# ctpeterson/qex

Hardware: AMD Instinct MI355X
Metric: staggered Dslash GFLOP/s + CG iters/s, 32^4 SU(3) fp64, 1/2/4/8 MI355X (higher is better)
Workload: dtype f64

## Files before the change

include/qexhip.h:

```cpp
#ifndef QEXHIP_H
#define QEXHIP_H

#include <stddef.h>

#ifdef __cplusplus
extern "C" {
#endif

typedef struct qexhip_ctx *qexhip_handle;

#define QEXHIP_OK 0
#define QEXHIP_ERR_ARG (-1)
#define QEXHIP_ERR_HIP (-2)
#define QEXHIP_ERR_STATE (-3)
#define QEXHIP_ERR_COMM (-4)
#define QEXHIP_ERR_IO (-5)

#define QEXHIP_EVEN 0
#define QEXHIP_ODD 1
#define QEXHIP_ALL 2

int qexhip_init(qexhip_handle *h, int device, const int latLocal[4],
                const int rankGeom[4], const int rankCoord[4]);
int qexhip_finalize(qexhip_handle h);
// ... 120 lines not shown
int qexhip_fat7_deriv(qexhip_handle h, const double *g, const double *dfl, const double coef[5], const double *dll, double naik, double *d);
int qexhip_hisq_force(qexhip_handle h, const double *g, const double *dsdsu, const double *dsdsul, double *f);
int qexhip_hisq_prepare(qexhip_handle h, const double *g, double *fl, double *ll);
int qexhip_hisq_closure_force(qexhip_handle h, const double *dsdsu, const double *dsdsul, double *f);
int qexhip_hisq_release(qexhip_handle h);
int qexhip_hisq_fermion_force(qexhip_handle h, double *f, const double *const *psi, const double *scale, int n);

int qexhip_stag_solve_xx_batch(qexhip_handle h, int n, double *const *x, const double *const *b, const double *mass,
                               const double *r2req, int maxits, int par_even, int *iters, double *r2_over_b2);
int qexhip_stag_solve_batch(qexhip_handle h, int n, double *const *x, const double *const *b, const double *mass,
                            const double *r2req, int maxits, int *iters, double *r2_over_b2);

int qexhip_stag_links_info(qexhip_handle h, int *nlinks, int *compressed, double *max_dev);
int qexhip_stag_links_storage(qexhip_handle h, int *bytes_per_link, long long *escaped);
int qexhip_link_residual_host(const double *links, int n, unsigned char *escaped, double *row2);
int qexhip_set_option(qexhip_handle h, const char *name, int value);

int qexhip_stag_set_links_hisq(qexhip_handle h, const double *g);
int qexhip_stag_set_links_nhyp(qexhip_handle h, const double *g, double alpha1, double alpha2, double alpha3,
                               const int antiperiodic[4], const int phases[4]);

int qexhip_nhyp_prepare(qexhip_handle h, const double *g, double alpha1, double alpha2, double alpha3, double *fl);
int qexhip_nhyp_force(qexhip_handle h, double *f, const double *chain);
int qexhip_nhyp_release(qexhip_handle h);
int qexhip_nhyp_gauge_force(qexhip_handle h, double *f, double cplaq, double crect, double cadjplaq);
int qexhip_nhyp_fforce(qexhip_handle h, double *f, int n, const double *const *phi, const double *mass, const double *scale,
                       const double *r2req, int maxits, const int antiperiodic[4], const int phases[4], int *iters);
int qexhip_nhyp_fermion_force(qexhip_handle h, double *f, const double *const *psi, const double *scale, int n,
                              const int antiperiodic[4], const int phases[4]);
int qexhip_nhyp_fforce_dev(qexhip_handle h, double *f, int n, const int *phi_ids, const double *mass, const double *scale,
// ... 55 lines not shown
```

qex_amd/__init__.py:

```python
from ._lib import QexHipError, LIB_PATH, lib
from .layout import Layout
from .gauge import setBC, stagPhase, rephase, unit, synthetic_random_su3, synthetic_gaussian_vector
from .staggered import (
    Context, device_count, Staggered, SolverParams, newStag, newStag3, link_residual_host, plaq, gaugeForce, gaugeFlow, gaugeSet, gaugeFlowResident, flowEQ, flowMeasure, gaugeAction, gaugeUpdate, reunit, wline, ploops, s4_gauge, ResidentMD, HisqCoefs, HypCoefs, makeImpLinks, fat7lDeriv, EVEN, ODD, ALL,
    SloppyNone, SloppySingle, SloppyHalf,
)
from .io import loadGauge, loadGaugeSlab, saveGauge, getFileLattice, gaugeFileInfo, writeField, readField, fileMetadata
from .rng import RngField, RngMilc6, MRG32k3a
from .mesons import stagLocalMesons, stagMesons, norm2slice, sft, printLocalMesons, pointSource, wallSource, localMesonTables
```

qex_amd/_lib.py:

```python
import ctypes as C
import os

_HERE = os.path.dirname(os.path.abspath(__file__))
LIB_PATH = os.environ.get("QEXHIP_LIB", os.path.join(_HERE, "libqexhip.so"))
_lib = None

_vp, _ci, _cd = C.c_void_p, C.c_int, C.c_double
_pi, _pd = C.POINTER(C.c_int), C.POINTER(C.c_double)
SYMBOLS = [
    ("qexhip_init", _ci, [C.POINTER(_vp), _ci, _pi, _pi, _pi]),
    ("qexhip_finalize", _ci, [_vp]),
    ("qexhip_device_count", _ci, [_pi]),
    ("qexhip_last_error", C.c_char_p, []),
    ("qexhip_sync", _ci, [_vp]),
    ("qexhip_device_info", _ci, [_vp, C.c_char_p, _ci]),
    ("qexhip_layout_default_inner", _ci, [_pi, _ci, _pi]),
    ("qexhip_layout_simd_map", _ci, [_pi, _pi, _pi]),
    ("qexhip_layout_vec_simd_to_v1", _ci, [_pi, _pi, _vp, _vp]),
    ("qexhip_layout_vec_v1_to_simd", _ci, [_pi, _pi, _vp, _vp]),
    ("qexhip_layout_gauge_simd_to_v1", _ci, [_pi, _pi, C.POINTER(C.c_void_p), _vp]),
    ("qexhip_layout_gauge_v1_to_simd", _ci, [_pi, _pi, _vp, C.POINTER(C.c_void_p)]),
    ("qexhip_comm_unique_id", _ci, [C.c_char_p]),
    ("qexhip_comm_init", _ci, [_vp, C.c_char_p, _ci, _ci]),
    ("qexhip_comm_force_halo", _ci, [_vp, _ci]),
# ... 46 lines not shown
    ("qexhip_plaq", _ci, [_vp, _vp]),
    ("qexhip_gauge_force", _ci, [_vp, _vp, _cd]),
    ("qexhip_wflow", _ci, [_vp, _ci, _cd]),
    ("qexhip_flow_EQ", _ci, [_vp, _ci, _vp]),
    ("qexhip_flow_measure", _ci, [_vp, _vp, _vp]),
    ("qexhip_gauge_force_general", _ci, [_vp, _vp, _cd, _cd, _ci]),
    ("qexhip_wflow_general", _ci, [_vp, _ci, _cd, _cd, _cd, _ci]),
    ("qexhip_fat7", _ci, [_vp, _vp, _pd, _vp, _vp, _cd]),
    ("qexhip_hisq_smear", _ci, [_vp, _vp, _vp, _vp]),
    ("qexhip_nhyp_smear", _ci, [_vp, _vp, _vp, _cd, _cd, _cd]),
    ("qexhip_stag_solve_xx_batch", _ci, [_vp, _ci, _vp, _vp, _vp, _vp, _ci, _ci, _pi, _vp]),
    ("qexhip_stag_solve_batch", _ci, [_vp, _ci, _vp, _vp, _vp, _vp, _ci, _pi, _vp]),
    ("qexhip_stag_links_info", _ci, [_vp, _pi, _pi, _vp]),
    ("qexhip_stag_links_storage", _ci, [_vp, _pi, C.POINTER(C.c_longlong)]),
    ("qexhip_link_residual_host", _ci, [_vp, _ci, _vp, _vp]),
    ("qexhip_set_option", _ci, [_vp, C.c_char_p, _ci]),
    ("qexhip_fat7_deriv", _ci, [_vp, _vp, _vp, _vp, _vp, _cd, _vp]),
    ("qexhip_hisq_force", _ci, [_vp, _vp, _vp, _vp, _vp]),
    ("qexhip_hisq_prepare", _ci, [_vp, _vp, _vp, _vp]),
    ("qexhip_hisq_closure_force", _ci, [_vp, _vp, _vp, _vp]),
    ("qexhip_hisq_release", _ci, [_vp]),
    ("qexhip_hisq_fermion_force", _ci, [_vp, _vp, _vp, _vp, _ci]),
    ("qexhip_stag_set_links_hisq", _ci, [_vp, _vp]),
    ("qexhip_stag_set_links_nhyp", _ci, [_vp, _vp, _cd, _cd, _cd, _pi, _pi]),
    ("qexhip_nhyp_prepare", _ci, [_vp, _vp, _cd, _cd, _cd, _vp]),
    ("qexhip_nhyp_force", _ci, [_vp, _vp, _vp]),
    ("qexhip_nhyp_release", _ci, [_vp]),
    ("qexhip_nhyp_fforce", _ci, [_vp, _vp, _ci, _vp, _vp, _vp, _vp, _ci, _pi, _pi, _pi]),
    ("qexhip_nhyp_gauge_force", _ci, [_vp, _vp, _cd, _cd, _cd]),
    ("qexhip_nhyp_fermion_force", _ci, [_vp, _vp, _vp, _vp, _ci, _pi, _pi]),
# ... 101 lines not shown
```

qex_amd/csrc/api.cpp:

```cpp
#include "qexhip_internal.h"
#include <string>
#include "../../include/qexhip.h"
#include <algorithm>
#include <cstdarg>
#include <cstdlib>
#include <cstring>
#include <vector>

static thread_local char g_err[1024] = "";

void qexhip_set_error(const char *fmt, ...) {
  va_list ap;
  va_start(ap, fmt);
  vsnprintf(g_err, sizeof(g_err), fmt, ap);
  va_end(ap);
}
extern "C" const char *qexhip_last_error(void) { return g_err; }

static bool timer_class_on(const qexhip_ctx *c, const char *name) {
  if (!c->timers_on) return false;
  if (c->timers_on == 2) return strncmp(name, "dslash", 6) == 0;
  if (c->timers_on == 3) return strncmp(name, "dslash", 6) == 0 || strcmp(name, "exchange") == 0 || strcmp(name, "allreduce") == 0;
  return true;
}
// ... 770 lines not shown
extern "C" int qexhip_stag_solve_batch(qexhip_handle c, int n, double *const *x, const double *const *b, const double *mass,
                                       const double *r2req, int maxits, int *iters, double *r2_over_b2) {
  if (!c || !x || !b || !mass || !r2req) return QEXHIP_ERR_ARG;
  HIPCHK(hipSetDevice(c->device));
  return solve_batch_host(c, n, x, b, mass, r2req, maxits, -1, iters, r2_over_b2);
}
extern "C" int qexhip_stag_links_info(qexhip_handle c, int *nlinks, int *compressed, double *max_dev) {
  if (!c) return QEXHIP_ERR_ARG;
  if (nlinks) *nlinks = c->W ? c->ndir : 0;
  if (compressed) *compressed = c->recon;
  if (max_dev) *max_dev = c->recon_dev;
  return 0;
}
extern "C" int qexhip_stag_links_storage(qexhip_handle c, int *bytes_per_link, long long *escaped) {
  if (!c) return QEXHIP_ERR_ARG;
  if (bytes_per_link) *bytes_per_link = !c->W ? 0 : (c->lres ? 108 : (c->recon == 1 ? 96 : (c->recon == 2 ? 112 : 144)));
  if (escaped) *escaped = c->lres_esc;
  return 0;
}
extern "C" int qexhip_link_residual_host(const double *links, int n, unsigned char *escaped, double *row2) {
  if (!links || n < 0) return QEXHIP_ERR_ARG;
  return link_residual_host((const double2 *)links, n, escaped, (double2 *)row2);
}
extern "C" int qexhip_hisq_prepare(qexhip_handle c, const double *g, double *fl, double *ll) {
  if (!c || !g) return QEXHIP_ERR_ARG;
  HIPCHK(hipSetDevice(c->device));
  return hisq_prepare(c, g, fl, ll);
}
extern "C" int qexhip_hisq_closure_force(qexhip_handle c, const double *dsdsu, const double *dsdsul, double *f) {
  if (!c || !dsdsu || !dsdsul || !f) return QEXHIP_ERR_ARG;
  HIPCHK(hipSetDevice(c->device));
  return hisq_closure_force(c, dsdsu, dsdsul, f);
}
extern "C" int qexhip_hisq_fermion_force(qexhip_handle c, double *f, const double *const *psi, const double *scale, int n) {
  if (!c || !f || !psi || !scale) return QEXHIP_ERR_ARG;
  HIPCHK(hipSetDevice(c->device));
  return hisq_fermion_force(c, f, psi, scale, n);
// ... 209 lines not shown
```

qex_amd/csrc/dslash.hip:

```cpp
#include "qexhip_internal.h"
#include "site_index.h"
#include "reduce.h"
#include "fused_sweep.h"
#include <hip/hip_ext.h>
#include <cstring>
#include <algorithm>
#include <chrono>

static double now_us() { return std::chrono::duration<double, std::micro>(std::chrono::steady_clock::now().time_since_epoch()).count(); }

struct DslashArgs {
  Geom g;
  const double2 *W;
  const unsigned long long *S;
  const double2 *in;
  double2 *out;
  const double2 *rin;
  const double2 *xs;
  double ca, cb;
  double sgn;
  double post;
  int parity, c0, c1;
  int d0, d1, nb1;
  const double2 *gh_hi, *gh_lo;
// ... 22 lines not shown
    if (A.swz && !bnd) {
      int per = A.swz >> 3;
      lb = (lb & 7) * per + (lb >> 3);
    }
    int c = A.c0 + lb * 256 + threadIdx.x;
    int clim = A.c1;
    if (FUSED) c = fused_site(A.fs, R, lb, A.c0, A.c1, A.d0, A.d1, clim);
    else if (lb >= A.nb1) { c = A.d0 + (lb - A.nb1) * 256 + threadIdx.x; clim = A.d1; }
    double dotv = 0;
    const bool active = c < clim && !skip;
    const Geom &g = A.g;
    const SiteXYZT s = site_coord(g, c, A.parity);
    const int tu = FUSED ? __builtin_amdgcn_readfirstlane(s.t) : 0;
    double2 acc[3];
    double2 xsv[3];
    constexpr int NLOAD = (RECON == 1 || RECON == 3) ? 6 : (RECON == 2 ? 7 : 9);
    constexpr int LROW = RECON == 3 ? LR_ROW : NLOAD * 64;
    const double2 *w = A.W + (size_t)(c >> 6) * (NDIR * LROW) + (c & 63);
    const unsigned long long *sm = RECON == 1 ? A.S + (size_t)(c >> 6) * NDIR : (RECON == 3 ? A.S + (size_t)(c >> 6) * NDIR * 2 : nullptr);
    const double2 *in_f1 = A.in, *in_b1 = A.in, *in_f3 = A.in, *in_b3 = A.in;
    if (FUSED) {
      in_f1 = tu + 1 >= g.X[3] ? A.gh_hi : A.in;
      in_b1 = tu - 1 < 0 ? A.gh_lo : A.in;
      in_f3 = tu + 3 >= g.X[3] ? A.gh_hi : A.in;
      in_b3 = tu - 3 < 0 ? A.gh_lo : A.in;
    }
    auto pair = [&](const int pr, const bool do_f, const bool do_b) __attribute__((always_inline)) {
      const int mu = pr & 3;
      const int hop = pr >= 4 ? 3 : 1;
      const int pf = nbr_pos<HALO>(g, c, s, mu, hop);
      const int pb = nbr_pos<HALO>(g, c, s, mu, -hop);
      const double2 *wp = w + (size_t)pr * (2 * LROW);
      double2 U[9], W[9], vf[3], vb[3];
      if (do_f) {
// ... 7 lines not shown
#pragma unroll
        for (int k = 0; k < NLOAD; k++) {
          d2v t = __builtin_nontemporal_load((const d2v *)&wp[LROW + k * 64]);
          W[k] = make_double2(t.x, t.y);
        }
      }
      if (RECON == 1) {
        const int lane = c & 63;
        if (do_f) recon_row2<1>(U, (sm[2 * pr] >> lane) & 1ull);
        if (do_b) recon_row2<1>(W, (sm[2 * pr + 1] >> lane) & 1ull);
      } else if (RECON == 3) {
        const int lane = c & 63;
        const size_t fr = ((size_t)(c >> 6) * NDIR + 2 * pr) * 576 + lane;
        if (do_f) recon_row2_res(U, wp - lane, sm + 4 * pr, A.S - 2, fr, lane);
        if (do_b) recon_row2_res(W, wp - lane + LROW, sm + 4 * pr + 2, A.S - 2, fr + 576, lane);
      } else if (RECON == 2) {
        if (do_f) recon_row2<2>(U, false);
        if (do_b) recon_row2<2>(W, false);
      }
      const double2 *srcf = (FUSED && mu == 3) ? (hop == 3 ? in_f3 : in_f1) : A.in;
      const double2 *srcb = (FUSED && mu == 3) ? (hop == 3 ? in_b3 : in_b1) : A.in;
      if (do_f) {
#pragma unroll
        for (int k = 0; k < 3; k++) vf[k] = srcf[vec_off(pf, k)];
      }
      if (do_b) {
#pragma unroll
        for (int k = 0; k < 3; k++) vb[k] = srcb[vec_off(pb, k)];
      }
      if (do_f) mv3<false>(acc, U, vf);
// ... 63 lines not shown
          acc[k].x *= (A.sgn * A.post); acc[k].y *= (A.sgn * A.post);
          if (A.ntstore) {
            d2v t; t.x = acc[k].x; t.y = acc[k].y;
            __builtin_nontemporal_store(t, (d2v *)&A.out[vec_off(c, k)]);
          } else {
            A.out[vec_off(c, k)] = acc[k];
          }
        }
        if (DOT) {
#pragma unroll
          for (int k = 0; k < 3; k++) dotv = fma(xsv[k].x, acc[k].x, fma(xsv[k].y, acc[k].y, dotv));
        }
      }
    }
    if (DOT && !skip && !parked) {
      const int pidx = !FUSED ? (RECON == 3 ? lb : (int)blockIdx.x) : fused_partial_slot(A.fs, R, lb);
      double r = block_sum_256(dotv);
      if (threadIdx.x == 0) A.partials[pidx] = r;
    }
    if (!cleanup) break;
  }
  if (FUSED) fused_finish(A.fs, R);
}

template <int NDIR, bool HALO, bool INIT, bool DOT, int RECON>
__global__ void __launch_bounds__(256) k_dslash(DslashArgs A) { dslash_body<NDIR, HALO, INIT, DOT, RECON, false>(A); }
template <int NDIR, bool INIT, bool DOT, int RECON>
__global__ void __launch_bounds__(256) k_dslash_fused(DslashArgs A) { dslash_body<NDIR, true, INIT, DOT, RECON, true>(A); }

template <class K>
static void launch_timed(qexhip_ctx *c, const char *tname, K kernel, dim3 grid, dim3 block, DslashArgs &A, hipStream_t st) {
// ... 21 lines not shown
#define QX_LAUNCH(R) \
  do { \
    if (HALO && fused) { \
      if (init && dot) launch_timed(c, tname, k_dslash_fused<NDIR, true, true, R>, grid, block, A, st); \
      else if (init) launch_timed(c, tname, k_dslash_fused<NDIR, true, false, R>, grid, block, A, st); \
      else if (dot) launch_timed(c, tname, k_dslash_fused<NDIR, false, true, R>, grid, block, A, st); \
      else launch_timed(c, tname, k_dslash_fused<NDIR, false, false, R>, grid, block, A, st); \
    } else if (init && dot) launch_timed(c, tname, k_dslash<NDIR, HALO, true, true, R>, grid, block, A, st); \
    else if (init) launch_timed(c, tname, k_dslash<NDIR, HALO, true, false, R>, grid, block, A, st); \
    else if (dot) launch_timed(c, tname, k_dslash<NDIR, HALO, false, true, R>, grid, block, A, st); \
    else launch_timed(c, tname, k_dslash<NDIR, HALO, false, false, R>, grid, block, A, st); \
  } while (0)
  if (c->recon == 1) QX_LAUNCH(1);
  else if (c->recon == 2) QX_LAUNCH(2);
  else if constexpr (NDIR == 8) {
    if (c->lres) QX_LAUNCH(3);
    else QX_LAUNCH(0);
  } else QX_LAUNCH(0);
#undef QX_LAUNCH
  A.partials = psave;
  HIPCHK(hipGetLastError());
  return 0;
}

void sweep_plan(const qexhip_ctx *c, int *lo_end_out, int *hi_beg_out, int *overlap_out) {
  const Geom &g = c->g;
  int lo_end = g.depth * g.F; if (lo_end > g.Vh) lo_end = g.Vh;
  int hi_beg = g.Vh - g.depth * g.F; if (hi_beg < lo_end) hi_beg = lo_end;
  const size_t face_bytes = (size_t)g.depth * g.F * 48;
  *lo_end_out = lo_end; *hi_beg_out = hi_beg;
  const int tuned = c->overlap_auto[c->ndir == 16];
// ... 4 lines not shown

int sweep_form(const qexhip_ctx *c, int overlap) {
  if (!overlap || !peer_faces(c)) return 0;
  if (c->opt_hop_split >= 0) return c->opt_hop_split ? 2 : 0;
  const int m = c->form_auto[c->ndir == 16];
  return m >= 0 ? m : 2;
}

static double exchange_estimate_us(const qexhip_ctx *c) {
  const double meas = c->xchg_us[c->ndir == 16];
  if (meas > 0) return meas;
  const double link = (c->emu_link_gbs > 0 ? c->emu_link_gbs : 45.0) * 1e3;
  return 3.0 + (double)c->g.depth * c->g.F * 48.0 / link;
}
double sweep_push_fraction(const qexhip_ctx *c, int interior_sites, int nrhs) {
  const double bsite = c->ndir * (c->recon == 1 ? 96.0 : (c->recon == 2 ? 112.0 : (c->lres ? 108.0 : 144.0))) + 120.0 * nrhs;
  const double t_int = (double)interior_sites * bsite / 5.5e6;
  return t_int > 0 ? std::min(1.0, std::max(0.65, nrhs * exchange_estimate_us(c) / t_int)) : 1.0;
}

static int sweep_fused_ctl(qexhip_ctx *c, int nbnd, FusedCtl *F, int nrhs) {
  if (c->fz_cap < nbnd) {
    HIPCHK(hipStreamSynchronize(c->stream));
    if (c->fz_buf) HIPCHK(hipFree(c->fz_buf));
    c->fz_buf = nullptr; c->fz_cap = 0;
    const int cap = std::max(2 * nbnd, 4096);
    HIPCHK(hipMalloc((void **)&c->fz_buf, (size_t)(256 + cap) * sizeof(unsigned int)));
    HIPCHK(hipMemsetAsync(c->fz_buf, 0, (size_t)(256 + cap) * sizeof(unsigned int), c->stream));
    c->fz_cap = cap;
  }
  F->dec = c->fz_buf; F->ndef = c->fz_buf + 32; F->cl_done = c->fz_buf + 64; F->late = c->fz_buf + 96;
// ... 96 lines not shown
  if (saved < 0) c->overlap_auto[slot] = (best > 0 && v[0] > 0 && best < 0.95 * v[0]) ? 1 : 0;
  for (int k = 0; k < 3; k++) c->overlap_tune_us[slot][k] = v[k] / 10.0;
  return 0;
}

int dslash_sweep(qexhip_ctx *c, DevField &out, DevField &in, int parity, const DslashOpts &o) {
  const Geom &g = c->g;
  if (!c->W) { qexhip_set_error("staggered links not set (qexhip_stag_set_links)"); return -3; }
  DslashArgs A;
  memset(&A, 0, sizeof A);
  A.g = g;
  if (c->recon) {
    A.W = c->Wc + (size_t)parity * g.ntile * c->ndir * (c->recon == 1 ? 384 : 448);
    A.S = c->Ws + (size_t)parity * g.ntile * c->ndir;
  } else if (c->lres) {
    A.W = c->Wc + (size_t)parity * g.ntile * c->ndir * LR_ROW;
    A.S = c->Wm + (size_t)parity * (2 + g.ntile * c->ndir * 2) + 2;
  } else {
    A.W = c->W + (size_t)parity * g.ntile * c->ndir * 576;
    A.S = nullptr;
  }
  A.in = in.par(1 - parity);
  A.out = out.par(parity);
  A.rin = o.rin ? o.rin->par(parity) : nullptr;
  A.xs = o.xs ? o.xs->par(parity) : nullptr;
  A.ca = o.ca; A.cb = o.cb;
  A.sgn = o.neg ? -1.0 : 1.0;
  A.post = o.post;
  A.parity = parity;
  A.partials = c->partials;
  A.done = o.done;
// ... 54 lines not shown
```

qex_amd/csrc/dslash_core.h:

```cpp
#pragma once
#include <hip/hip_runtime.h>
#include "link_residual.h"

typedef double d2v __attribute__((ext_vector_type(2)));

template <bool SUB>
__device__ __forceinline__ void mv3(double2 acc[3], const double2 U[9], const double2 v[3]) {
#pragma unroll
  for (int i = 0; i < 3; i++) {
#pragma unroll
    for (int j = 0; j < 3; j++) {
      if (!SUB) {
        acc[i].x += U[3 * i + j].x * v[j].x;
        acc[i].x -= U[3 * i + j].y * v[j].y;
        acc[i].y += U[3 * i + j].x * v[j].y;
        acc[i].y += U[3 * i + j].y * v[j].x;
      } else {
        acc[i].x -= U[3 * i + j].x * v[j].x;
        acc[i].x += U[3 * i + j].y * v[j].y;
        acc[i].y -= U[3 * i + j].x * v[j].y;
        acc[i].y -= U[3 * i + j].y * v[j].x;
      }
    }
  }
// ... 24 lines not shown
__device__ __forceinline__ void recon_row2_res(double2 U[9], const double2 *row, const unsigned long long *m, const unsigned long long *hdr,
                                               size_t fr, int lane) {
  const uint64_t lo = __builtin_nontemporal_load((const uint64_t *)(row + LR_RES) + lane);
  const uint32_t hi = __builtin_nontemporal_load((const uint32_t *)(row + LR_RES + 32) + lane);
  double2 r2[3];
  lr_decode(U, (m[0] >> lane) & 1ull, lo, hi, r2);
  if ((m[1] >> lane) & 1ull) {
    const double2 *wf = (const double2 *)(uintptr_t)hdr[0] + fr;
#pragma unroll
    for (int k = 0; k < 3; k++) r2[k] = wf[(6 + k) * 64];
  }
#pragma unroll
  for (int k = 0; k < 3; k++) U[6 + k] = r2[k];
}

template <int RECON>
__device__ __forceinline__ void load_link(double2 U[9], const double2 *w, const unsigned long long *sm, int lane) {
  constexpr int NLOAD = RECON == 1 ? 6 : (RECON == 2 ? 7 : 9);
#pragma unroll
  for (int k = 0; k < NLOAD; k++) U[k] = w[k * 64];
  if (RECON == 1) recon_row2<1>(U, (*sm >> lane) & 1ull);
  else if (RECON == 2) recon_row2<2>(U, false);
}
```

qex_amd/csrc/layout.hip:

```cpp
#include <algorithm>
#include <vector>
#include "qexhip_internal.h"
#include "site_index.h"
#include "link_residual.h"
#include <cstring>

int geom_init(Geom &g, const int X[4], int depth, int halo) {
  for (int i = 0; i < 4; i++) {
    if (X[i] < 2 || (X[i] & 1)) { qexhip_set_error("local lattice extents must be even and >= 2 (got %d in dim %d)", X[i], i); return -1; }
    if (X[i] > 1024) { qexhip_set_error("local lattice extents above 1024 are not supported (got %d in dim %d)", X[i], i); return -1; }
    g.X[i] = X[i];
  }
  g.Xh = X[0] / 2;
  g.V = X[0] * X[1] * X[2] * X[3];
  g.Vh = g.V / 2;
  g.F = g.Xh * X[1] * X[2];
  g.ntile = (g.Vh + QEXHIP_TILE - 1) / QEXHIP_TILE;
  g.halo = halo;
  g.depth = halo ? depth : 0;
  if (halo) {
    if (g.F % QEXHIP_TILE) { qexhip_set_error("sharding in t needs X*Y*Z/2 to be a multiple of 64 (got %d)", g.F); return -1; }
    if (X[3] < 3) { qexhip_set_error("sharding in t needs a local t extent >= 3"); return -1; }
    g.gtile = 3 * g.F / QEXHIP_TILE;
  } else {
// ... 196 lines not shown
  bool neg;
  uint64_t lo;
  uint32_t hi;
  const bool ok = lr_encode(u, &neg, &lo, &hi);
  ((uint64_t *)(Wc + row * LR_ROW + LR_RES))[l] = lo;
  ((uint32_t *)(Wc + row * LR_ROW + LR_RES + 32))[l] = hi;
  const unsigned long long sgn = __ballot(neg), esc = __ballot(!ok);
  if (l == 0) {
    unsigned long long *m = Wm + 2 * (row + row / prows + 1);
    m[0] = sgn;
    m[1] = esc;
    if (esc) atomicAdd(nesc, (unsigned int)__popcll(esc));
  }
}

int link_residual_host(const double2 *u, long n, unsigned char *escaped, double2 *row2) {
  for (long i = 0; i < n; i++) {
    bool neg;
    uint64_t lo;
    uint32_t hi;
    const bool ok = lr_encode(u + 9 * i, &neg, &lo, &hi);
    if (escaped) escaped[i] = !ok;
    if (row2) lr_decode(u + 9 * i, neg, lo, hi, row2 + 3 * i);
  }
  return 0;
}

int links_compress(qexhip_ctx *c) {
  const Geom &g = c->g;
  c->links_gen++;
  c->recon = 0;
  c->lres = 0; c->lres_esc = 0;
  if (!c->opt_recon || !c->W) return 0;
  const size_t nrows = (size_t)2 * g.ntile * c->ndir;
  if (c->Wc_rows < nrows) {
    if (c->Wc) HIPCHK(hipFree(c->Wc));
    if (c->Ws) HIPCHK(hipFree(c->Ws));
    HIPCHK(hipMalloc((void **)&c->Wc, nrows * 448 * sizeof(double2)));
// ... 4 lines not shown
  const unsigned nblk = (unsigned)((nrows * 64 + 255) / 256);
  for (int fmt = 1; fmt <= 2; fmt++) {
    if (fmt == 2 && c->opt_recon == 1) break;
    HIPCHK(hipMemsetAsync(flag, 0, sizeof(unsigned int), c->stream));
    if (fmt == 1) k_links_compress<1><<<nblk, 256, 0, c->stream>>>(nrows, c->W, c->Wc, c->Ws, flag);
    else k_links_compress<2><<<nblk, 256, 0, c->stream>>>(nrows, c->W, c->Wc, c->Ws, flag);
    HIPCHK(hipGetLastError());
    unsigned int bits = 0;
    HIPCHK(hipMemcpyAsync(&bits, flag, sizeof(bits), hipMemcpyDeviceToHost, c->stream));
    HIPCHK(hipStreamSynchronize(c->stream));
    float dev;
    memcpy(&dev, &bits, sizeof(dev));
    if (fmt == 1 || dev <= 5e-14f) c->recon_dev = dev;
    if (dev <= 5e-14f) { c->recon = fmt; break; }
  }
  if (!c->recon && c->opt_lossless && c->ndir == 8) {
    if (!c->Wm || c->Wm_rows < nrows) {
      if (c->Wm) HIPCHK(hipFree(c->Wm));
      c->Wm = nullptr; c->Wm_rows = 0;
      HIPCHK(hipMalloc((void **)&c->Wm, (nrows + 2) * 2 * sizeof(unsigned long long)));
      c->Wm_rows = nrows;
    }
    const size_t prows = nrows / 2;
    HIPCHK(hipMemsetAsync(flag, 0, sizeof(unsigned int), c->stream));
    k_links_residual<<<nblk, 256, 0, c->stream>>>(nrows, prows, c->W, c->Wc, c->Wm, flag);
    HIPCHK(hipGetLastError());
    unsigned int nesc = 0;
    HIPCHK(hipMemcpyAsync(&nesc, flag, sizeof(nesc), hipMemcpyDeviceToHost, c->stream));
    const unsigned long long hdr[2][2] = {{(unsigned long long)(uintptr_t)c->W, 0}, {(unsigned long long)(uintptr_t)(c->W + prows * 576), 0}};
    for (int p = 0; p < 2; p++) HIPCHK(hipMemcpyAsync(c->Wm + p * 2 * (prows + 1), hdr[p], sizeof hdr[p], hipMemcpyHostToDevice, c->stream));
    HIPCHK(hipStreamSynchronize(c->stream));
    c->lres_esc = nesc;
    if ((double)nesc <= 0.01 * (double)(nrows * 64)) c->lres = 1;
  }
  return 0;
}

__global__ void __launch_bounds__(256) k_links_from_nat(Geom g, const double2 *__restrict__ N, double2 *W, int ndir, int dbase, int hop) {
  int i = blockIdx.x * 256 + threadIdx.x;
  if (i >= g.V) return;
  int p = i >= g.Vh, c = i - p * g.Vh;
  SiteXYZT s = site_coord(g, c, p);
  double2 *w = W + ((size_t)p * g.ntile + (c >> 6)) * ndir * 576 + (c & 63);
  for (int mu = 0; mu < 4; mu++) {
    const double2 *U = N + (((size_t)p * g.etile + (c >> 6)) * 4 + mu) * 576 + (c & 63);
    double2 *wf = w + (size_t)(dbase + 2 * mu) * 576;
    for (int k = 0; k < 9; k++) wf[k * 64] = U[k * 64];
    int cb;
// ... 167 lines not shown
```

qex_amd/csrc/qexhip_internal.h:

```cpp
#pragma once
#include <hip/hip_runtime.h>
#include <cstdint>
#include <cstdio>
#include <string>
#include <vector>
#include <map>

#define QEXHIP_TILE 64

struct Geom {
  int X[4];
  int Xh;
  int V, Vh;
  int F;
  int ntile;
  int depth;
  int gtile;
  int etile;
  int halo;
};

__host__ __device__ inline size_t vec_off(int pos, int colour) {
  return (size_t)(pos >> 6) * 192 + (size_t)colour * 64 + (size_t)(pos & 63);
}
// ... 68 lines not shown
  int next_field = 1;
  double *stage = nullptr; size_t stage_bytes = 0;
  double *partials = nullptr; int npartials = 0;
  int part2_off = 0;
  double *dscal = nullptr;
  CgScal *cg = nullptr;
  struct { int valid = 0; const double2 *x = nullptr; int par_even = 0; double m2 = 0; int k = 0; } cg_resume;
  int cg_r2parts = 0;
  double *hist = nullptr; int histcap = 0;
  void *pinned = nullptr;
  int wk[WK_SLOTS]{0};
  int timers_on = 0;
  std::map<std::string, TimerSlot> timers;
  double2 *Wc = nullptr; unsigned long long *Ws = nullptr; size_t Wc_rows = 0; int recon = 0; double recon_dev = 0;
  unsigned long long *Wm = nullptr; size_t Wm_rows = 0; int lres = 0; long long lres_esc = 0;
  int opt_lossless = 1;
  int opt_batch_multi = 0;
  int opt_multi_reduce = 0;
  int opt_force_pair = 1;
  int opt_obs_clover = 1;
  int opt_hop_split = -1;
  int opt_fused_spin_us = -1;
  int ranks_share_device = 0;
  int hybrid_sums = 0;
  unsigned int *fz_buf = nullptr; int fz_cap = 0;
  const double2 *bnd_out_on_cstream = nullptr;
  double xchg_us[2]{0, 0};
  int form_auto[2]{-1, -1};
  int opt_chain_overlap = 1;
  int opt_smear_ca = 1;
  int opt_flow_exp = 1;
// ... 38 lines not shown
  ScopedTimer(qexhip_ctx *c_, const char *name, hipStream_t st_);
  ~ScopedTimer();
};
int timers_collect(qexhip_ctx *c);
bool timer_event_pair(qexhip_ctx *c, const char *name, hipEvent_t *e0, hipEvent_t *e1);

int geom_init(Geom &g, const int X[4], int depth, int halo);
int field_alloc(qexhip_ctx *c, DevField &f);
int field_upload(qexhip_ctx *c, DevField &f, const double *host);
int field_download(qexhip_ctx *c, const DevField &f, double *host);
int links_upload(qexhip_ctx *c, const double *fat, const double *lng);
int ensure_stage(qexhip_ctx *c, size_t bytes);
int links_from_natural(qexhip_ctx *c, const double2 *fat, const double2 *lng);
int links_compress(qexhip_ctx *c);
int link_residual_host(const double2 *u, long n, unsigned char *escaped, double2 *row2);
int op_eo_reconstruct_pub(qexhip_ctx *c, DevField &r, DevField &b, double m);
int op_eo_reduce_pub(qexhip_ctx *c, DevField &r, DevField &b, double m);
int op_stagD_pub(qexhip_ctx *c, DevField &r, DevField &x, int parity, double m, double sc, double a);
void batch_state_free(qexhip_ctx *c);
int batch_io_fields(qexhip_ctx *c, int n, DevField **xs, DevField **bs);
int solve_full_batch_dev(qexhip_ctx *c, int n, DevField **x, DevField **b, const double *mass, const double *r2req,
                         int maxits, int *iters, double *r2_final);
int nhyp_fforce(qexhip_ctx *c, double *f_host, int n, const double *const *phi, const double *mass, const double *scale,
                const double *r2req, int maxits, int bcmask, const int ph[4], int *iters, DevField *const *phi_dev = nullptr);
int solve_batch_host(qexhip_ctx *c, int n, double *const *x, const double *const *b, const double *mass,
                     const double *r2req, int maxits, int xx_parity, int *iters, double *r2);

inline bool multi_rank(const qexhip_ctx *c) { return c->nranks > 1 || c->opt_multi_reduce; }

int comm_halo_push_only_multi(qexhip_ctx *c, int n, DevField *const *f, int parity, const double2 **gh_hi, const double2 **gh_lo, struct PeerPush *push);
// ... 162 lines not shown
```

qex_amd/staggered.py:

```python
import ctypes as C
import time
import numpy as np

from . import _lib
from ._lib import check, lib

EVEN, ODD, ALL = 0, 1, 2
SloppyNone, SloppySingle, SloppyHalf = 0, 1, 2
_SUBSET = {"even": EVEN, "odd": ODD, "all": ALL}


def _p(a):
    if a is None:
        return None
    if a.dtype != np.float64 or not a.flags["C_CONTIGUOUS"]:
        raise ValueError("fields must be C-contiguous float64 arrays")
    return a.ctypes.data_as(C.c_void_p)


class SolverParams:

    def __init__(self, r2req=1e-6, maxits=50000, verbosity=1, usePrevSoln=False, sloppySolve=SloppyNone):
        self.r2req = r2req
        self.maxits = maxits
# ... 445 lines not shown
    return Staggered(ctx, g, g3)


def link_residual_host(links):
    a = np.asarray(links)
    if np.iscomplexobj(a):
        a = np.stack([a.real, a.imag], axis=-1)
    a = np.ascontiguousarray(a, dtype=np.float64).reshape(-1, 18)
    n = a.shape[0]
    esc = np.zeros(n, dtype=np.uint8)
    row2 = np.zeros((n, 3, 2), dtype=np.float64)
    check(lib().qexhip_link_residual_host(a.ctypes.data, n, esc.ctypes.data, row2.ctypes.data))
    return esc.astype(bool), row2


def plaq(ctx, g=None):
    if g is not None:
        check(lib().qexhip_gauge_set(ctx._h, _p(g)))
    out = np.zeros(6)
    check(lib().qexhip_plaq(ctx._h, _p(out)))
    return out


_FLOW_KIND = {"Wilson": 0, "rect": 0, "adj": 1}


def gaugeForce(ctx, g, cplaq=1.0, rect=0.0, adjplaq=0.0):
    if rect != 0.0 and adjplaq != 0.0:
        raise ValueError("rect and adjplaq are separate code paths in QEX (gaugeForce vs forceA)")
    check(lib().qexhip_gauge_set(ctx._h, _p(g)))
# ... 218 lines not shown
```

Baseline: 2806.

## Add second lossless link-compression format reconstructing rows 0-1 from unitarity

Adds a new lossless residual link encoding (lres=2) that stores only 4 complex entries plus three 64-bit residual words per link (88 bytes instead of 108). Rows 0 and 1 are partly reconstructed from unitarity constraints using Newton sqrt and reciprocal iterations, with 16-bit integer corrections that make the result bit-exact, and row 2 is rebuilt with the existing residual decoder. Links that do not round-trip exactly fall back to the uncompressed copy through escape masks. This is made the default, with a fallback to format 1 when too many links escape. The aim is less link memory traffic in the bandwidth-bound Dslash, paid for with more FP64 arithmetic per link and some divergence on escaped links.

```diff
diff --git a/include/qexhip.h b/include/qexhip.h
--- a/include/qexhip.h
+++ b/include/qexhip.h
@@ -158,6 +158,7 @@
 int qexhip_stag_links_info(qexhip_handle h, int *nlinks, int *compressed, double *max_dev);
 int qexhip_stag_links_storage(qexhip_handle h, int *bytes_per_link, long long *escaped);
 int qexhip_link_residual_host(const double *links, int n, unsigned char *escaped, double *row2);
+int qexhip_link_residual2_host(const double *links, int n, unsigned char *escaped, double *decoded, unsigned long long *words);
 int qexhip_set_option(qexhip_handle h, const char *name, int value);
 
 int qexhip_stag_set_links_hisq(qexhip_handle h, const double *g);
diff --git a/qex_amd/__init__.py b/qex_amd/__init__.py
--- a/qex_amd/__init__.py
+++ b/qex_amd/__init__.py
@@ -2,7 +2,7 @@
 from .layout import Layout
 from .gauge import setBC, stagPhase, rephase, unit, synthetic_random_su3, synthetic_gaussian_vector
 from .staggered import (
-    Context, device_count, Staggered, SolverParams, newStag, newStag3, link_residual_host, plaq, gaugeForce, gaugeFlow, gaugeSet, gaugeFlowResident, flowEQ, flowMeasure, gaugeAction, gaugeUpdate, reunit, wline, ploops, s4_gauge, ResidentMD, HisqCoefs, HypCoefs, makeImpLinks, fat7lDeriv, EVEN, ODD, ALL,
+    Context, device_count, Staggered, SolverParams, newStag, newStag3, link_residual_host, link_residual2_host, plaq, gaugeForce, gaugeFlow, gaugeSet, gaugeFlowResident, flowEQ, flowMeasure, gaugeAction, gaugeUpdate, reunit, wline, ploops, s4_gauge, ResidentMD, HisqCoefs, HypCoefs, makeImpLinks, fat7lDeriv, EVEN, ODD, ALL,
     SloppyNone, SloppySingle, SloppyHalf,
 )
 from .io import loadGauge, loadGaugeSlab, saveGauge, getFileLattice, gaugeFileInfo, writeField, readField, fileMetadata
diff --git a/qex_amd/_lib.py b/qex_amd/_lib.py
--- a/qex_amd/_lib.py
+++ b/qex_amd/_lib.py
@@ -84,6 +84,7 @@
     ("qexhip_stag_links_info", _ci, [_vp, _pi, _pi, _vp]),
     ("qexhip_stag_links_storage", _ci, [_vp, _pi, C.POINTER(C.c_longlong)]),
     ("qexhip_link_residual_host", _ci, [_vp, _ci, _vp, _vp]),
+    ("qexhip_link_residual2_host", _ci, [_vp, _ci, _vp, _vp, _vp]),
     ("qexhip_set_option", _ci, [_vp, C.c_char_p, _ci]),
     ("qexhip_fat7_deriv", _ci, [_vp, _vp, _vp, _vp, _vp, _cd, _vp]),
     ("qexhip_hisq_force", _ci, [_vp, _vp, _vp, _vp, _vp]),
diff --git a/qex_amd/csrc/api.cpp b/qex_amd/csrc/api.cpp
--- a/qex_amd/csrc/api.cpp
+++ b/qex_amd/csrc/api.cpp
@@ -808,13 +808,17 @@
 }
 extern "C" int qexhip_stag_links_storage(qexhip_handle c, int *bytes_per_link, long long *escaped) {
   if (!c) return QEXHIP_ERR_ARG;
-  if (bytes_per_link) *bytes_per_link = !c->W ? 0 : (c->lres ? 108 : (c->recon == 1 ? 96 : (c->recon == 2 ? 112 : 144)));
+  if (bytes_per_link) *bytes_per_link = !c->W ? 0 : (c->lres ? (c->lres == 2 ? 88 : 108) : (c->recon == 1 ? 96 : (c->recon == 2 ? 112 : 144)));
   if (escaped) *escaped = c->lres_esc;
   return 0;
 }
 extern "C" int qexhip_link_residual_host(const double *links, int n, unsigned char *escaped, double *row2) {
   if (!links || n < 0) return QEXHIP_ERR_ARG;
   return link_residual_host((const double2 *)links, n, escaped, (double2 *)row2);
+}
+extern "C" int qexhip_link_residual2_host(const double *links, int n, unsigned char *escaped, double *decoded, unsigned long long *words) {
+  if (!links || n < 0) return QEXHIP_ERR_ARG;
+  return link_residual2_host((const double2 *)links, n, escaped, (double2 *)decoded, words);
 }
 extern "C" int qexhip_hisq_prepare(qexhip_handle c, const double *g, double *fl, double *ll) {
   if (!c || !g) return QEXHIP_ERR_ARG;
diff --git a/qex_amd/csrc/dslash.hip b/qex_amd/csrc/dslash.hip
--- a/qex_amd/csrc/dslash.hip
+++ b/qex_amd/csrc/dslash.hip
@@ -60,10 +60,10 @@
     const int tu = FUSED ? __builtin_amdgcn_readfirstlane(s.t) : 0;
     double2 acc[3];
     double2 xsv[3];
-    constexpr int NLOAD = (RECON == 1 || RECON == 3) ? 6 : (RECON == 2 ? 7 : 9);
-    constexpr int LROW = RECON == 3 ? LR_ROW : NLOAD * 64;
+    constexpr int NLOAD = RECON == 4 ? 4 : ((RECON == 1 || RECON == 3) ? 6 : (RECON == 2 ? 7 : 9));
+    constexpr int LROW = RECON == 4 ? LR2_ROW : (RECON == 3 ? LR_ROW : NLOAD * 64);
     const double2 *w = A.W + (size_t)(c >> 6) * (NDIR * LROW) + (c & 63);
-    const unsigned long long *sm = RECON == 1 ? A.S + (size_t)(c >> 6) * NDIR : (RECON == 3 ? A.S + (size_t)(c >> 6) * NDIR * 2 : nullptr);
+    const unsigned long long *sm = RECON == 1 ? A.S + (size_t)(c >> 6) * NDIR : (RECON >= 3 ? A.S + (size_t)(c >> 6) * NDIR * 2 : nullptr);
     const double2 *in_f1 = A.in, *in_b1 = A.in, *in_f3 = A.in, *in_b3 = A.in;
     if (FUSED) {
       in_f1 = tu + 1 >= g.X[3] ? A.gh_hi : A.in;
@@ -101,6 +101,11 @@
         const size_t fr = ((size_t)(c >> 6) * NDIR + 2 * pr) * 576 + lane;
         if (do_f) recon_row2_res(U, wp - lane, sm + 4 * pr, A.S - 2, fr, lane);
         if (do_b) recon_row2_res(W, wp - lane + LROW, sm + 4 * pr + 2, A.S - 2, fr + 576, lane);
+      } else if (RECON == 4) {
+        const int lane = c & 63;
+        const size_t fr = ((size_t)(c >> 6) * NDIR + 2 * pr) * 576 + lane;
+        if (do_f) recon_link_res2(U, wp - lane, sm + 4 * pr, A.S - 2, fr, lane);
+        if (do_b) recon_link_res2(W, wp - lane + LROW, sm + 4 * pr + 2, A.S - 2, fr + 576, lane);
       } else if (RECON == 2) {
         if (do_f) recon_row2<2>(U, false);
         if (do_b) recon_row2<2>(W, false);
@@ -194,7 +199,7 @@
       }
     }
     if (DOT && !skip && !parked) {
-      const int pidx = !FUSED ? (RECON == 3 ? lb : (int)blockIdx.x) : fused_partial_slot(A.fs, R, lb);
+      const int pidx = !FUSED ? (RECON >= 3 ? lb : (int)blockIdx.x) : fused_partial_slot(A.fs, R, lb);
       double r = block_sum_256(dotv);
       if (threadIdx.x == 0) A.partials[pidx] = r;
     }
@@ -246,7 +251,8 @@
   if (c->recon == 1) QX_LAUNCH(1);
   else if (c->recon == 2) QX_LAUNCH(2);
   else if constexpr (NDIR == 8) {
-    if (c->lres) QX_LAUNCH(3);
+    if (c->lres == 2) QX_LAUNCH(4);
+    else if (c->lres) QX_LAUNCH(3);
     else QX_LAUNCH(0);
   } else QX_LAUNCH(0);
 #undef QX_LAUNCH
@@ -281,7 +287,7 @@
   return 3.0 + (double)c->g.depth * c->g.F * 48.0 / link;
 }
 double sweep_push_fraction(const qexhip_ctx *c, int interior_sites, int nrhs) {
-  const double bsite = c->ndir * (c->recon == 1 ? 96.0 : (c->recon == 2 ? 112.0 : (c->lres ? 108.0 : 144.0))) + 120.0 * nrhs;
+  const double bsite = c->ndir * (c->recon == 1 ? 96.0 : (c->recon == 2 ? 112.0 : (c->lres ? (c->lres == 2 ? 88.0 : 108.0) : 144.0))) + 120.0 * nrhs;
   const double t_int = (double)interior_sites * bsite / 5.5e6;
   return t_int > 0 ? std::min(1.0, std::max(0.65, nrhs * exchange_estimate_us(c) / t_int)) : 1.0;
 }
@@ -408,7 +414,7 @@
     A.W = c->Wc + (size_t)parity * g.ntile * c->ndir * (c->recon == 1 ? 384 : 448);
     A.S = c->Ws + (size_t)parity * g.ntile * c->ndir;
   } else if (c->lres) {
-    A.W = c->Wc + (size_t)parity * g.ntile * c->ndir * LR_ROW;
+    A.W = c->Wc + (size_t)parity * g.ntile * c->ndir * (c->lres == 2 ? LR2_ROW : LR_ROW);
     A.S = c->Wm + (size_t)parity * (2 + g.ntile * c->ndir * 2) + 2;
   } else {
     A.W = c->W + (size_t)parity * g.ntile * c->ndir * 576;
diff --git a/qex_amd/csrc/dslash_core.h b/qex_amd/csrc/dslash_core.h
--- a/qex_amd/csrc/dslash_core.h
+++ b/qex_amd/csrc/dslash_core.h
@@ -1,6 +1,7 @@
 #pragma once
 #include <hip/hip_runtime.h>
 #include "link_residual.h"
+#include "link_residual2.h"
 
 typedef double d2v __attribute__((ext_vector_type(2)));
 
@@ -62,6 +63,39 @@
   for (int k = 0; k < 3; k++) U[6 + k] = r2[k];
 }
 
+__device__ __forceinline__ void recon_link_res2(double2 U[9], const double2 *row, const unsigned long long *m, const unsigned long long *hdr,
+                                                size_t fr, int lane) {
+  typedef unsigned long long u2v __attribute__((ext_vector_type(2)));
+  const u2v wa = __builtin_nontemporal_load((const u2v *)(row + LR2_WA) + lane);
+  const uint64_t wb = __builtin_nontemporal_load((const uint64_t *)(row + LR2_WB) + lane);
+  const double2 st[4] = {U[0], U[1], U[2], U[3]};
+  uint32_t sel = (uint32_t)(wb >> 32);
+  uint64_t kw = wa.x;
+  double2 ap, bp, bq;
+  lr2_rows01<false>(st, &sel, &kw, &ap, &bp, &bq, nullptr, nullptr);
+  int p, q, r;
+  lr2_cols(sel, &p, &q, &r);
+  const double2 *wf = (const double2 *)(uintptr_t)hdr[0] + fr;
+  if ((m[0] >> lane) & 1ull) {
+    ap = wf[p * 64];
+    bp = wf[(3 + p) * 64];
+    bq = wf[(3 + q) * 64];
+  }
+#pragma unroll
+  for (int j = 0; j < 3; j++) {
+    U[j] = j == p ? ap : (j == q ? st[0] : st[1]);
+    U[3 + j] = j == p ? bp : (j == q ? bq : st[2]);
+  }
+  double2 r2[3];
+  lr_decode(U, (sel >> 7) & 1, wa.y, (uint32_t)wb, r2);
+  if ((m[1] >> lane) & 1ull) {
+#pragma unroll
+    for (int k = 0; k < 3; k++) r2[k] = wf[(6 + k) * 64];
+  }
+#pragma unroll
+  for (int k = 0; k < 3; k++) U[6 + k] = r2[k];
+}
+
 template <int RECON>
 __device__ __forceinline__ void load_link(double2 U[9], const double2 *w, const unsigned long long *sm, int lane) {
   constexpr int NLOAD = RECON == 1 ? 6 : (RECON == 2 ? 7 : 9);
diff --git a/qex_amd/csrc/layout.hip b/qex_amd/csrc/layout.hip
--- a/qex_amd/csrc/layout.hip
+++ b/qex_amd/csrc/layout.hip
@@ -3,6 +3,7 @@
 #include "qexhip_internal.h"
 #include "site_index.h"
 #include "link_residual.h"
+#include "link_residual2.h"
 #include <cstring>
 
 int geom_init(Geom &g, const int X[4], int depth, int halo) {
@@ -234,6 +235,34 @@
   }
 }
 
+__global__ void __launch_bounds__(256) k_links_residual2(size_t nrows, size_t prows, const double2 *__restrict__ W, double2 *Wc,
+                                                         unsigned long long *Wm, unsigned int *nesc) {
+  const size_t j = (size_t)blockIdx.x * 256 + threadIdx.x;
+  const size_t row = j >> 6;
+  if (row >= nrows) return;
+  const int l = j & 63;
+  const double2 *w = W + row * 576 + l;
+  double2 *o = Wc + row * LR2_ROW;
+  double2 u[9], st[4];
+#pragma unroll
+  for (int k = 0; k < 9; k++) u[k] = w[k * 64];
+  uint64_t wa[2], wb;
+  bool e01, e2;
+  lr2_encode(u, st, wa, &wb, &e01, &e2);
+#pragma unroll
+  for (int k = 0; k < 4; k++) o[k * 64 + l] = st[k];
+  ((uint64_t *)(o + LR2_WA))[2 * l] = wa[0];
+  ((uint64_t *)(o + LR2_WA))[2 * l + 1] = wa[1];
+  ((uint64_t *)(o + LR2_WB))[l] = wb;
+  const unsigned long long m01 = __ballot(e01), m2 = __ballot(e2);
+  if (l == 0) {
+    unsigned long long *m = Wm + 2 * (row + row / prows + 1);
+    m[0] = m01;
+    m[1] = m2;
+    if (m01 | m2) atomicAdd(nesc, (unsigned int)__popcll(m01 | m2));
+  }
+}
+
 int link_residual_host(const double2 *u, long n, unsigned char *escaped, double2 *row2) {
   for (long i = 0; i < n; i++) {
     bool neg;
@@ -242,6 +271,24 @@
     const bool ok = lr_encode(u + 9 * i, &neg, &lo, &hi);
     if (escaped) escaped[i] = !ok;
     if (row2) lr_decode(u + 9 * i, neg, lo, hi, row2 + 3 * i);
+  }
+  return 0;
+}
+
+int link_residual2_host(const double2 *u, long n, unsigned char *escaped, double2 *dec, unsigned long long *words) {
+  for (long i = 0; i < n; i++) {
+    double2 st[4];
+    uint64_t wa[2], wb;
+    bool e01, e2;
+    lr2_encode(u + 9 * i, st, wa, &wb, &e01, &e2);
+    if (escaped) escaped[i] = (unsigned char)((e01 ? 1 : 0) | (e2 ? 2 : 0));
+    if (dec) {
+      int p, q, r;
+      lr2_cols((uint32_t)(wb >> 32), &p, &q, &r);
+      const double2 ex[3] = {u[9 * i + p], u[9 * i + 3 + p], u[9 * i + 3 + q]};
+      lr2_decode(st, wa[0], wa[1], wb, e01 ? ex : nullptr, dec + 9 * i);
+    }
+    if (words) { words[3 * i] = wa[0]; words[3 * i + 1] = wa[1]; words[3 * i + 2] = wb; }
   }
   return 0;
 }
@@ -276,7 +323,7 @@
     if (fmt == 1 || dev <= 5e-14f) c->recon_dev = dev;
     if (dev <= 5e-14f) { c->recon = fmt; break; }
   }
-  if (!c->recon && c->opt_lossless && c->ndir == 8) {
+  if (!c->recon && c->opt_lossless > 0 && c->ndir == 8) {
     if (!c->Wm || c->Wm_rows < nrows) {
       if (c->Wm) HIPCHK(hipFree(c->Wm));
       c->Wm = nullptr; c->Wm_rows = 0;
@@ -284,16 +331,19 @@
       c->Wm_rows = nrows;
     }
     const size_t prows = nrows / 2;
-    HIPCHK(hipMemsetAsync(flag, 0, sizeof(unsigned int), c->stream));
-    k_links_residual<<<nblk, 256, 0, c->stream>>>(nrows, prows, c->W, c->Wc, c->Wm, flag);
-    HIPCHK(hipGetLastError());
-    unsigned int nesc = 0;
-    HIPCHK(hipMemcpyAsync(&nesc, flag, sizeof(nesc), hipMemcpyDeviceToHost, c->stream));
-    const unsigned long long hdr[2][2] = {{(unsigned long long)(uintptr_t)c->W, 0}, {(unsigned long long)(uintptr_t)(c->W + prows * 576), 0}};
-    for (int p = 0; p < 2; p++) HIPCHK(hipMemcpyAsync(c->Wm + p * 2 * (prows + 1), hdr[p], sizeof hdr[p], hipMemcpyHostToDevice, c->stream));
-    HIPCHK(hipStreamSynchronize(c->stream));
-    c->lres_esc = nesc;
-    if ((double)nesc <= 0.01 * (double)(nrows * 64)) c->lres = 1;
+    for (int fmt = c->opt_lossless >= 2 ? 2 : 1; fmt >= 1 && !c->lres; fmt--) {
+      HIPCHK(hipMemsetAsync(flag, 0, sizeof(unsigned int), c->stream));
+      if (fmt == 2) k_links_residual2<<<nblk, 256, 0, c->stream>>>(nrows, prows, c->W, c->Wc, c->Wm, flag);
+      else k_links_residual<<<nblk, 256, 0, c->stream>>>(nrows, prows, c->W, c->Wc, c->Wm, flag);
+      HIPCHK(hipGetLastError());
+      unsigned int nesc = 0;
+      HIPCHK(hipMemcpyAsync(&nesc, flag, sizeof(nesc), hipMemcpyDeviceToHost, c->stream));
+      const unsigned long long hdr[2][2] = {{(unsigned long long)(uintptr_t)c->W, 0}, {(unsigned long long)(uintptr_t)(c->W + prows * 576), 0}};
+      for (int p = 0; p < 2; p++) HIPCHK(hipMemcpyAsync(c->Wm + p * 2 * (prows + 1), hdr[p], sizeof hdr[p], hipMemcpyHostToDevice, c->stream));
+      HIPCHK(hipStreamSynchronize(c->stream));
+      c->lres_esc = nesc;
+      if ((double)nesc <= 0.01 * (double)(nrows * 64)) c->lres = fmt;
+    }
   }
   return 0;
 }
diff --git a/qex_amd/csrc/link_residual2.h b/qex_amd/csrc/link_residual2.h
--- /dev/null
+++ b/qex_amd/csrc/link_residual2.h
@@ -0,0 +1,203 @@
+#pragma once
+#include "link_residual.h"
+
+#define LR2_ROW 352
+#define LR2_WA 256
+#define LR2_WB 320
+
+__host__ __device__ __forceinline__ double lr2_csign(double m, double s) {
+  return lr_double(lr_bits(m) | (lr_bits(s) & 0x8000000000000000ull));
+}
+
+__host__ __device__ __forceinline__ double lr2_sqrt(double d) {
+#pragma clang fp contract(off)
+  const bool pos = d > 0;
+  const double dd = pos ? d : 1.0;
+  double y = lr_double(0x5fe6eb50c7b537a9ull - (lr_bits(dd) >> 1));
+  const double h = 0.5 * dd;
+#pragma unroll
+  for (int i = 0; i < 4; i++) {
+    const double r = y * y;
+    const double e = fma(-h, r, 0.5);
+    y = fma(y, e, y);
+  }
+  return pos ? dd * y : 0.0;
+}
+
+__host__ __device__ __forceinline__ double lr2_recip(double d) {
+#pragma clang fp contract(off)
+  const uint64_t b = lr_bits(d);
+  double y = lr_double((0x7fde623822fc16e6ull - (b & 0x7fffffffffffffffull)) | (b & 0x8000000000000000ull));
+#pragma unroll
+  for (int i = 0; i < 3; i++) {
+    const double e = fma(-d, y, 1.0);
+    y = fma(y, fma(e, e, e), y);
+  }
+  return y;
+}
+
+__host__ __device__ __forceinline__ int lr2_k(uint64_t w, int j) { return (int16_t)(w >> (16 * j)); }
+
+__host__ __device__ __forceinline__ int lr2_res(double rec, double tru, bool *ok) {
+  const double sc = lr_double(lr_bits(rec) & 0x7ff0000000000000ull) * 0x1p-52;
+  const double qv = sc > 0 ? (tru - rec) / sc : 0.0;
+  int k = fabs(qv) <= 32767.0 ? (int)rint(qv) : 0;
+  if (lr_bits(lr_apply(rec, k)) != lr_bits(tru)) { k = 0; *ok = false; }
+  return k;
+}
+
+template <bool ENC>
+__host__ __device__ __forceinline__ void lr2_rows01(const double2 st[4], uint32_t *sel, uint64_t *kw, double2 *ap, double2 *bp,
+                                                    double2 *bq, const double2 *tru, bool *ok) {
+#pragma clang fp contract(off)
+  const uint32_t s = *sel;
+  const bool h0 = (s >> 3) & 1, h1 = (s >> 4) & 1, sg = (s >> 5) & 1;
+  const double2 aq = st[0], ar = st[1], br = st[2];
+  const double ao = st[3].x, bo = st[3].y;
+  int k[4] = {0, 0, 0, 0};
+  if (!ENC) {
+#pragma unroll
+    for (int j = 0; j < 4; j++) k[j] = lr2_k(*kw, j);
+  }
+  double n0 = ao * ao;
+  n0 = fma(aq.x, aq.x, n0);
+  n0 = fma(aq.y, aq.y, n0);
+  n0 = fma(ar.x, ar.x, n0);
+  n0 = fma(ar.y, ar.y, n0);
+  double x = lr2_sqrt(1.0 - n0);
+  x = sg ? -x : x;
+  if (ENC) { k[0] = lr2_res(x, h0 ? tru[0].y : tru[0].x, ok); x = h0 ? tru[0].y : tru[0].x; }
+  else x = lr_apply(x, k[0]);
+  const double2 a_p = h0 ? make_double2(ao, x) : make_double2(x, ao);
+  double P = a_p.x * a_p.x;
+  P = fma(a_p.y, a_p.y, P);
+  const double2 bq0 = h1 ? make_double2(bo, 0.0) : make_double2(0.0, bo);
+  double tx = ar.x * br.x;
+  tx = fma(ar.y, br.y, tx);
+  tx = fma(aq.x, bq0.x, tx);
+  tx = fma(aq.y, bq0.y, tx);
+  double ty = ar.x * br.y;
+  ty = fma(-ar.y, br.x, ty);
+  ty = fma(aq.x, bq0.y, ty);
+  ty = fma(-aq.y, bq0.x, ty);
+  const double cx = h1 ? aq.y : aq.x, cy = h1 ? aq.x : -aq.y;
+  double be = tx * cx;
+  be = fma(ty, cy, be);
+  double al = aq.x * aq.x;
+  al = fma(aq.y, aq.y, al);
+  al = al + P;
+  double s0 = bo * bo;
+  s0 = fma(br.x, br.x, s0);
+  s0 = fma(br.y, br.y, s0);
+  double ga = tx * tx;
+  ga = fma(ty, ty, ga);
+  ga = fma(P, s0 - 1.0, ga);
+  double dq = be * be;
+  dq = fma(-al, ga, dq);
+  const double t = be + lr2_csign(lr2_sqrt(dq), be);
+  double y;
+  if (ENC) {
+    const double ya = -(t * lr2_recip(al)), yb = -(ga * lr2_recip(t));
+    const double yt = h1 ? tru[2].y : tru[2].x;
+    const bool rt = fabs(yt - yb) < fabs(yt - ya);
+    *sel = s | (rt ? 64u : 0u);
+    y = rt ? yb : ya;
+    k[1] = lr2_res(y, yt, ok);
+    y = yt;
+  } else {
+    const bool rt = (s >> 6) & 1;
+    const double num = rt ? ga : t, den = rt ? t : al;
+    y = -(num * lr2_recip(den));
+    y = lr_apply(y, k[1]);
+  }
+  *bq = h1 ? make_double2(bo, y) : make_double2(y, bo);
+  tx = fma(y, cx, tx);
+  ty = fma(y, cy, ty);
+  const double iP = lr2_recip(P);
+  double mx = tx * a_p.x;
+  mx = fma(-ty, a_p.y, mx);
+  double my = tx * a_p.y;
+  my = fma(ty, a_p.x, my);
+  double2 b_p = make_double2(-(mx * iP), -(my * iP));
+  if (ENC) {
+    k[2] = lr2_res(b_p.x, tru[1].x, ok);
+    k[3] = lr2_res(b_p.y, tru[1].y, ok);
+    b_p = tru[1];
+    *kw = (uint64_t)(uint16_t)k[0] | (uint64_t)(uint16_t)k[1] << 16 | (uint64_t)(uint16_t)k[2] << 32 | (uint64_t)(uint16_t)k[3] << 48;
+  } else {
+    b_p = make_double2(lr_apply(b_p.x, k[2]), lr_apply(b_p.y, k[3]));
+  }
+  *ap = a_p;
+  *bp = b_p;
+}
+
+__host__ __device__ __forceinline__ void lr2_cols(uint32_t sel, int *p, int *q, int *r) {
+  const int pp = sel & 3, qq = (pp + 1 + ((sel >> 2) & 1)) % 3;
+  *p = pp; *q = qq; *r = 3 - pp - qq;
+}
+
+__host__ __device__ __forceinline__ void lr2_encode(const double2 u[9], double2 st[4], uint64_t wa[2], uint64_t *wb, bool *esc01,
+                                                   bool *esc2) {
+  const double r0[6] = {u[0].x, u[0].y, u[1].x, u[1].y, u[2].x, u[2].y};
+  const double r1[6] = {u[3].x, u[3].y, u[4].x, u[4].y, u[5].x, u[5].y};
+  bool fin = true;
+#pragma unroll
+  for (int j = 0; j < 9; j++) fin = fin && fabs(u[j].x) <= 1.7976931348623157e308 && fabs(u[j].y) <= 1.7976931348623157e308;
+  int m0 = 0;
+#pragma unroll
+  for (int j = 1; j < 6; j++) m0 = fabs(r0[j]) > fabs(r0[m0]) ? j : m0;
+  const int p = m0 >> 1, h0 = m0 & 1;
+  const int c1 = (p + 1) % 3, c2 = (p + 2) % 3;
+  const double cand[4] = {r1[2 * c1], r1[2 * c1 + 1], r1[2 * c2], r1[2 * c2 + 1]};
+  int m1 = 0;
+#pragma unroll
+  for (int j = 1; j < 4; j++) m1 = fabs(cand[j]) > fabs(cand[m1]) ? j : m1;
+  const int qf = m1 >> 1, h1 = m1 & 1;
+  const int q = qf ? c2 : c1, r = 3 - p - q;
+  uint32_t sel = (uint32_t)p | (uint32_t)qf << 2 | (uint32_t)h0 << 3 | (uint32_t)h1 << 4 | (uint32_t)(lr_bits(r0[m0]) >> 63) << 5;
+  st[0] = u[q];
+  st[1] = u[r];
+  st[2] = u[3 + r];
+  st[3] = make_double2(h0 ? u[p].x : u[p].y, h1 ? u[3 + q].x : u[3 + q].y);
+  const double2 tru[3] = {u[p], u[3 + p], u[3 + q]};
+  bool ok = fin;
+  uint64_t kw = 0;
+  double2 ap, bp, bq;
+  lr2_rows01<true>(st, &sel, &kw, &ap, &bp, &bq, tru, &ok);
+  if (ok) {
+    uint64_t kd = kw;
+    lr2_rows01<false>(st, &sel, &kd, &ap, &bp, &bq, nullptr, nullptr);
+    ok = lr_bits(ap.x) == lr_bits(tru[0].x) && lr_bits(ap.y) == lr_bits(tru[0].y) && lr_bits(bp.x) == lr_bits(tru[1].x) &&
+         lr_bits(bp.y) == lr_bits(tru[1].y) && lr_bits(bq.x) == lr_bits(tru[2].x) && lr_bits(bq.y) == lr_bits(tru[2].y);
+  }
+  if (!ok) kw = 0;
+  bool neg;
+  uint64_t lo;
+  uint32_t hi;
+  const bool ok2 = lr_encode(u, &neg, &lo, &hi) && fin;
+  wa[0] = kw;
+  wa[1] = ok2 ? lo : 0;
+  *wb = (uint64_t)(ok2 ? hi : 0u) | (uint64_t)(sel | (neg ? 128u : 0u)) << 32;
+  *esc01 = !ok;
+  *esc2 = !ok2;
+}
+
+__host__ __device__ __forceinline__ void lr2_decode(const double2 st[4], uint64_t wa0, uint64_t wa1, uint64_t wb, const double2 *rows01,
+                                                   double2 u[9]) {
+  uint32_t sel = (uint32_t)(wb >> 32);
+  uint64_t kw = wa0;
+  double2 ap, bp, bq;
+  lr2_rows01<false>(st, &sel, &kw, &ap, &bp, &bq, nullptr, nullptr);
+  if (rows01) { ap = rows01[0]; bp = rows01[1]; bq = rows01[2]; }
+  int p, q, r;
+  lr2_cols(sel, &p, &q, &r);
+#pragma unroll
+  for (int j = 0; j < 3; j++) {
+    u[j] = j == p ? ap : (j == q ? st[0] : st[1]);
+    u[3 + j] = j == p ? bp : (j == q ? bq : st[2]);
+  }
+  double2 r2[3];
+  lr_decode(u, (sel >> 7) & 1, wa1, (uint32_t)wb, r2);
+#pragma unroll
+  for (int j = 0; j < 3; j++) u[6 + j] = r2[j];
+}
diff --git a/qex_amd/csrc/qexhip_internal.h b/qex_amd/csrc/qexhip_internal.h
--- a/qex_amd/csrc/qexhip_internal.h
+++ b/qex_amd/csrc/qexhip_internal.h
@@ -106,7 +106,7 @@
   std::map<std::string, TimerSlot> timers;
   double2 *Wc = nullptr; unsigned long long *Ws = nullptr; size_t Wc_rows = 0; int recon = 0; double recon_dev = 0;
   unsigned long long *Wm = nullptr; size_t Wm_rows = 0; int lres = 0; long long lres_esc = 0;
-  int opt_lossless = 1;
+  int opt_lossless = 2;
   int opt_batch_multi = 0;
   int opt_multi_reduce = 0;
   int opt_force_pair = 1;
@@ -175,6 +175,7 @@
 int links_from_natural(qexhip_ctx *c, const double2 *fat, const double2 *lng);
 int links_compress(qexhip_ctx *c);
 int link_residual_host(const double2 *u, long n, unsigned char *escaped, double2 *row2);
+int link_residual2_host(const double2 *u, long n, unsigned char *escaped, double2 *dec, unsigned long long *words);
 int op_eo_reconstruct_pub(qexhip_ctx *c, DevField &r, DevField &b, double m);
 int op_eo_reduce_pub(qexhip_ctx *c, DevField &r, DevField &b, double m);
 int op_stagD_pub(qexhip_ctx *c, DevField &r, DevField &x, int parity, double m, double sc, double a);
diff --git a/qex_amd/staggered.py b/qex_amd/staggered.py
--- a/qex_amd/staggered.py
+++ b/qex_amd/staggered.py
@@ -483,6 +483,19 @@
     return esc.astype(bool), row2
 
 
+def link_residual2_host(links):
+    a = np.asarray(links)
+    if np.iscomplexobj(a):
+        a = np.stack([a.real, a.imag], axis=-1)
+    a = np.ascontiguousarray(a, dtype=np.float64).reshape(-1, 18)
+    n = a.shape[0]
+    esc = np.zeros(n, dtype=np.uint8)
+    dec = np.zeros((n, 3, 3, 2), dtype=np.float64)
+    words = np.zeros((n, 3), dtype=np.uint64)
+    check(lib().qexhip_link_residual2_host(a.ctypes.data, n, esc.ctypes.data, dec.ctypes.data, words.ctypes.data))
+    return esc, dec, words
+
+
 def plaq(ctx, g=None):
     if g is not None:
         check(lib().qexhip_gauge_set(ctx._h, _p(g)))
```

Result: no change. 2818 (median of 5 runs) (+0.4%).
